# AO33/HiC_Genome_Assembler

Hardware: AMD Instinct MI355X
Metric: Part1+Part2 wall-clock (s) and bins/s on N x N contact map (higher is better)
Workload: dtype f64

## Files before the change

hic_genome_assembler_amd/csrc/k_part2_window.hip:

```cpp
#include <cstdlib>

#include "hicmi_internal.h"

namespace hicmi {

__device__ __forceinline__ double wave_sum_w(double v)
{
#pragma unroll
    for (int off = 32; off >= 1; off >>= 1) v += __shfl_xor(v, off, 64);
    return v;
}

static constexpr int WT_SLICES = 64;
static constexpr int WT_UNIT = 160;
__host__ __device__ inline int64_t wt_q_size(int k) { return ((int64_t)k * 2) << k; }
__host__ __device__ inline int64_t wt_p_size(int k) { return ((int64_t)k * k * 4) << k; }
int64_t window_table_doubles(int k) { return WT_SLICES * wt_q_size(k) + wt_p_size(k) + 8; }

__host__ __device__ inline void wt_split(int Lj, int m, int n_out, int& nrg, int& nq)
{
    const int nr = Lj > 0 ? (Lj + 15) >> 4 : 1, tiles_w = ((((m + 15) >> 4) + 3) >> 2);
    const int64_t work = (int64_t)nr * tiles_w * ((n_out + 3) >> 2);
    int64_t units = (work + WT_UNIT - 1) / WT_UNIT;
    units = units < 1 ? 1 : (units > WT_SLICES ? WT_SLICES : units);
    nrg = nr < (int)units ? nr : (int)units;
    nq = (int)units / nrg;
    const int by_cols = n_out >= 64 ? n_out / 32 : 1;
    nq = nq > by_cols ? by_cols : nq;
    nq = nq < 1 ? 1 : nq;
}

static constexpr int WT_ACC = 8;

__device__ __forceinline__ int spread_bit(int v, int b) { return ((v >> b) << (b + 1)) | (v & ((1 << b) - 1)); }

template <bool H_IN_LDS>
__global__ __launch_bounds__(256) void k_win_outside(const double* __restrict__ M2, int64_t ld2,
                                                     const int32_t* __restrict__ pos2sel, int n, int k,
                                                     const WindowBatchEntry* __restrict__ wb, const double* H,
                                                     double* __restrict__ tables, int64_t table_stride)
{
    extern __shared__ __attribute__((aligned(16))) unsigned char smem_w[];
    __shared__ int s_len[8], s_glen[256];
    const WindowBatchEntry& we = wb[blockIdx.y];
    const int j = blockIdx.x, p0 = we.p0, m = we.m;
    const int tid = threadIdx.x, lane = tid & 63, wave = tid >> 6;
    int nrg, nq;
    wt_split(we.w.len[j], m, n - m, nrg, nq);
    if ((int)blockIdx.z >= nrg * nq) return;
    if (tid < k) s_len[tid] = we.w.len[tid];
    const double hn = H[n - 1];
    if (H_IN_LDS) {
        double* hl = reinterpret_cast<double*>(smem_w);
        for (int i = tid; i < n; i += 256) hl[i] = H[i];
        H = hl;
    }
    __syncthreads();
    if (tid < (1 << k)) {
        int g = 0;
        for (int b = 0; b < k; b++) if ((tid >> b) & 1) g += s_len[b];
        s_glen[tid] = g;
    }
    __syncthreads();
    const int Lj = s_len[j], startj = we.w.start[j], n_out = n - m;
    const int rt = blockIdx.z % nrg, qs = blockIdx.z / nrg;
    const int q_lo = (int)(((int64_t)qs * n_out) / nq), q_hi = (int)(((int64_t)(qs + 1) * n_out) / nq);
    double* __restrict__ Q = tables + (int64_t)blockIdx.y * table_stride + blockIdx.z * wt_q_size(k) + (((int64_t)j * 2) << k);
    const int n_entries = 2 << (k - 1);
    for (int e0 = wave * WT_ACC; e0 < n_entries; e0 += 4 * WT_ACC) {
        double acc[WT_ACC];
        int off[WT_ACC], rev[WT_ACC];
#pragma unroll
        for (int u = 0; u < WT_ACC; u++) {
            const int e = e0 + u < n_entries ? e0 + u : n_entries - 1;
            rev[u] = e >> (k - 1);
            off[u] = p0 + s_glen[spread_bit(e & ((1 << (k - 1)) - 1), j)];
            acc[u] = 0.0;
        }
        for (int i = rt * 16; i < Lj; i = (i & 15) == 15 ? i + 1 + (nrg - 1) * 16 : i + 1) {
            const double* __restrict__ row = M2 + (int64_t)(startj + i) * ld2;
#pragma unroll 2
            for (int qq = q_lo + lane; qq < q_hi; qq += 64) {
                const int pos = qq < p0 ? qq : qq + m;
                const double v = row[pos2sel[pos]];
#pragma unroll
                for (int u = 0; u < WT_ACC; u++) {
                    const int slot = off[u] + (rev[u] ? Lj - 1 - i : i);
                    const int d = slot > pos ? slot - pos : pos - slot;
                    acc[u] += v * (hn - H[d - 1]);
                }
            }
        }
#pragma unroll
        for (int u = 0; u < WT_ACC; u++) {
            const double sum = wave_sum_w(acc[u]);
            const int e = e0 + u;
            if (lane == 0 && e < n_entries)
                Q[((int64_t)(e >> (k - 1)) << k) | spread_bit(e & ((1 << (k - 1)) - 1), j)] = sum;
        }
    }
}

typedef double mfma_d4 __attribute__((ext_vector_type(4)));
static constexpr int WM_QC = 128;
static constexpr int WM_MAX_TILES = 8;

template <bool H_IN_LDS, int TILES>
__global__ __launch_bounds__(256) void k_win_outside_mfma(const double* __restrict__ M2, int64_t ld2,
                                                          const int32_t* __restrict__ pos2sel, int n, int k,
                                                          const WindowBatchEntry* __restrict__ wb, const double* H,
                                                          double* __restrict__ tables, int64_t table_stride, int m_pad_max)
{
    extern __shared__ __attribute__((aligned(16))) unsigned char smem_w[];
    double* As = reinterpret_cast<double*>(smem_w);
    double* Gt = As;
    const int as_doubles = 16 * (WM_QC + 1) > 16 * m_pad_max ? 16 * (WM_QC + 1) : 16 * m_pad_max;
    __shared__ int s_len[8], s_glen[256], s_pos[WM_QC], s_col[WM_QC];
    const WindowBatchEntry& we = wb[blockIdx.y];
    const int j = blockIdx.x, p0 = we.p0, m = we.m;
    const int tid = threadIdx.x, lane = tid & 63, wave = tid >> 6;
    int nrg, nq;
    wt_split(we.w.len[j], m, n - m, nrg, nq);
    if ((int)blockIdx.z >= nrg * nq) return;
    if (tid < k) s_len[tid] = we.w.len[tid];
    const double hn = H[n - 1];
    if (H_IN_LDS) {
        double* hl = As + as_doubles;
        for (int i = tid; i < n; i += 256) hl[i] = H[i];
        H = hl;
    }
    __syncthreads();
    if (tid < (1 << k)) {
        int g = 0;
        for (int b = 0; b < k; b++) if ((tid >> b) & 1) g += s_len[b];
        s_glen[tid] = g;
    }
    __syncthreads();
    const int Lj = s_len[j], startj = we.w.start[j], n_out = n - m;
    const int rt = blockIdx.z % nrg, qs = blockIdx.z / nrg;
    const int q_lo = (int)(((int64_t)qs * n_out) / nq), q_hi = (int)(((int64_t)(qs + 1) * n_out) / nq);
    double* __restrict__ Q = tables + (int64_t)blockIdx.y * table_stride + blockIdx.z * wt_q_size(k) + (((int64_t)j * 2) << k);
    const int n_entries = 2 << (k - 1);
    const int m_pad = (m + 15) & ~15, n_tiles = m_pad >> 4;
    const int e_rev = tid < n_entries ? tid >> (k - 1) : 0;
    const int e_off = tid < n_entries ? s_glen[spread_bit(tid & ((1 << (k - 1)) - 1), j)] : 0;
    double qacc = 0.0;
    for (int r0 = rt * 16; r0 < Lj; r0 += nrg * 16) {
        mfma_d4 acc[TILES];
#pragma unroll
        for (int t = 0; t < TILES; t++) acc[t] = mfma_d4{0.0, 0.0, 0.0, 0.0};
        for (int qc = q_lo; qc < q_hi; qc += WM_QC) {
            const int cols = q_hi - qc < WM_QC ? q_hi - qc : WM_QC;
            if (q_hi - q_lo > WM_QC || r0 == rt * 16) {
                __syncthreads();
                if (tid < WM_QC) {
                    const int qq = qc + tid;
                    const int pos = tid < cols ? (qq < p0 ? qq : qq + m) : -1;
                    s_pos[tid] = pos;
                    s_col[tid] = pos >= 0 ? pos2sel[pos] : 0;
                }
            }
            __syncthreads();
            {
                constexpr int RPT = 16 * WM_QC / 256;
                const int cq = tid % WM_QC, rb = (tid / WM_QC) * RPT;
                const int c = s_col[cq];
                const bool okc = cq < cols;
                double v[RPT];
#pragma unroll
                for (int r = 0; r < RPT; r++)
                    v[r] = okc && r0 + rb + r < Lj ? M2[(int64_t)(startj + r0 + rb + r) * ld2 + c] : 0.0;
#pragma unroll
                for (int r = 0; r < RPT; r++) As[(rb + r) * (WM_QC + 1) + cq] = v[r];
            }
            __syncthreads();
            const int kk_end = (cols + 3) >> 2;
#pragma unroll 2
            for (int kk = 0; kk < kk_end; kk++) {
                const int kq = kk * 4 + (lane >> 4);
                const double a = As[(lane & 15) * (WM_QC + 1) + kq];
                int pos = s_pos[kq];
                pos = pos < 0 ? p0 : pos;
#pragma unroll
                for (int t = 0; t < TILES; t++) {
                    const int st = wave + 4 * t;
                    if (st < n_tiles) {
                        int d = p0 + st * 16 + (lane & 15) - pos;
                        d = d < 0 ? -d : d;
                        d = d < 1 ? 1 : (d > n - 1 ? n - 1 : d);
                        const double b = hn - H[d - 1];
                        acc[t] = __builtin_amdgcn_mfma_f64_16x16x4f64(a, b, acc[t], 0, 0, 0);
                    }
                }
            }
        }
        __syncthreads();
#pragma unroll
        for (int t = 0; t < TILES; t++) {
            const int st = wave + 4 * t;
            if (st < n_tiles) {
#pragma unroll
                for (int r = 0; r < 4; r++) Gt[((lane >> 4) + 4 * r) * m_pad_max + st * 16 + (lane & 15)] = acc[t][r];
            }
        }
        __syncthreads();
        if (tid < n_entries) {
            const int rows = Lj - r0 < 16 ? Lj - r0 : 16;
            for (int r = 0; r < rows; r++) {
                const int i = r0 + r;
                qacc += Gt[r * m_pad_max + e_off + (e_rev ? Lj - 1 - i : i)];
            }
        }
        __syncthreads();
    }
    if (tid < n_entries) Q[((int64_t)e_rev << k) | spread_bit(tid & ((1 << (k - 1)) - 1), j)] = qacc;
}

template <bool H_IN_LDS>
__global__ __launch_bounds__(256) void k_win_pairs(const double* __restrict__ M2, int64_t ld2, int n, int k,
                                                   const WindowBatchEntry* __restrict__ wb, const double* H,
                                                   double* __restrict__ tables, int64_t table_stride)
{
    extern __shared__ __attribute__((aligned(16))) unsigned char smem_w[];
    __shared__ int s_len[8], s_glen[256];
    __shared__ double s_part[4];
    const WindowBatchEntry& we = wb[blockIdx.y];
    const int a = blockIdx.x / k, b = blockIdx.x - a * k, m = we.m;
    const int tid = threadIdx.x, lane = tid & 63, wave = tid >> 6;
    if (tid < k) s_len[tid] = we.w.len[tid];
    const double hn = H[n - 1];
    if (H_IN_LDS) {
        double* hl = reinterpret_cast<double*>(smem_w);
        for (int i = tid; i < m; i += 256) hl[i] = H[i];
        H = hl;
    }
    __syncthreads();
    if (tid < (1 << k)) {
        int g = 0;
        for (int c = 0; c < k; c++) if ((tid >> c) & 1) g += s_len[c];
        s_glen[tid] = g;
    }
    __syncthreads();
    double* __restrict__ base = tables + (int64_t)blockIdx.y * table_stride;
    const int La = s_len[a], starta = we.w.start[a];
    if (a == b) {
        double acc = 0.0;
        const int pairs = La * La;
        for (int flat = tid; flat < pairs; flat += 256) {
            const int e = flat / La, f = flat - e * La;
            if (f > e) acc += M2[(int64_t)(starta + e) * ld2 + starta + f] * (hn - H[f - e - 1]);
        }
        acc = wave_sum_w(acc);
        if (lane == 0) s_part[wave] = acc;
        __syncthreads();
        if (tid == 0) base[WT_SLICES * wt_q_size(k) + wt_p_size(k) + a] = (s_part[0] + s_part[1]) + (s_part[2] + s_part[3]);
        int nrg, nq;
        wt_split(La, m, n - m, nrg, nq);
        const int nz = nrg * nq;
        const int64_t q_size = wt_q_size(k);
        for (int e = tid; e < (2 << k) && nz > 1; e += 256) {
            if ((e >> a) & 1) continue;
            double* __restrict__ q0 = base + (((int64_t)a * 2) << k) + e;
            double sum = q0[0];
            for (int z = 1; z < nz; z++) sum += q0[z * q_size];
            q0[0] = sum;
        }
        return;
    }
    const int Lb = s_len[b], startb = we.w.start[b];
    const int lo = a < b ? a : b, hi = a < b ? b : a;
    double* __restrict__ P = base + WT_SLICES * wt_q_size(k) + ((((int64_t)a * k + b) * 4) << k);
    const int n_sets = k >= 2 ? 1 << (k - 2) : 1, n_entries = 4 * n_sets, pairs = La * Lb;
    for (int e0 = wave * WT_ACC; e0 < n_entries; e0 += 4 * WT_ACC) {
        double acc[WT_ACC];
        int gap[WT_ACC], ra[WT_ACC], rb[WT_ACC];
#pragma unroll
        for (int u = 0; u < WT_ACC; u++) {
            const int e = e0 + u < n_entries ? e0 + u : n_entries - 1;
            const int orient = e / n_sets, set = e - orient * n_sets;
            ra[u] = orient >> 1; rb[u] = orient & 1;
            gap[u] = s_glen[spread_bit(spread_bit(set, lo), hi)];
            acc[u] = 0.0;
        }
#pragma unroll 2
        for (int flat = lane; flat < pairs; flat += 64) {
            const int ea = flat / Lb, eb = flat - ea * Lb;
            const double v = M2[(int64_t)(starta + ea) * ld2 + startb + eb];
#pragma unroll
            for (int u = 0; u < WT_ACC; u++) {
                const int i = ra[u] ? La - 1 - ea : ea, jj = rb[u] ? Lb - 1 - eb : eb;
                const int d = La - i + gap[u] + jj;
                acc[u] += v * (hn - H[d - 1]);
            }
        }
#pragma unroll
        for (int u = 0; u < WT_ACC; u++) {
            const double sum = wave_sum_w(acc[u]);
            const int e = e0 + u;
            if (lane == 0 && e < n_entries) {
                const int orient = e / n_sets, set = e - orient * n_sets;
                P[((int64_t)orient << k) | spread_bit(spread_bit(set, lo), hi)] = sum;
            }
        }
    }
}

__global__ __launch_bounds__(256) void k_win_candidates(int k, const int8_t* __restrict__ orders,
                                                        const uint8_t* __restrict__ orients, int n_ori, int n_cand,
                                                        const double* __restrict__ tables, int64_t table_stride,
                                                        double* __restrict__ delta_all)
{
    const int c = blockIdx.x * 256 + threadIdx.x;
    if (c >= n_cand) return;
    const double* __restrict__ base = tables + (int64_t)blockIdx.y * table_stride;
    const double* __restrict__ Q = base;
    const int64_t q_size = wt_q_size(k);
    const double* __restrict__ P = base + WT_SLICES * q_size;
    const double* __restrict__ C = P + wt_p_size(k);
    const int8_t* __restrict__ ord = orders + (int64_t)(c / n_ori) * k;
    const uint8_t* __restrict__ ori = orients + (int64_t)(c % n_ori) * k;
    double sum = 0.0;
    for (int j = 0; j < k; j++) sum += C[j];
    int before = 0;
    for (int s = 0; s < k; s++) {
        const int a = ord[s], ra = ori[s] ? 1 : 0;
        const int64_t qi = ((int64_t)(a * 2 + ra) << k) | before;
        sum += Q[qi];
        int between = 0;
        for (int t = s + 1; t < k; t++) {
            const int b = ord[t], rb = ori[t] ? 1 : 0;
            sum += P[((((int64_t)a * k + b) * 4 + ra * 2 + rb) << k) | between];
            between |= 1 << b;
        }
        before |= 1 << a;
    }
    delta_all[(int64_t)blockIdx.y * n_cand + c] = sum;
}

static constexpr int NL_ITERS = 32;
static constexpr int NL_ORDERS = 4 * NL_ITERS;
static inline int64_t stride_of(int k) { return window_table_doubles(k); }

template <bool LIST>
__global__ __launch_bounds__(256) void k_win_near(int k, const int8_t* __restrict__ orders, const uint8_t* __restrict__ orients,
                                                  int n_ord, int n_ori, const double* __restrict__ tables, int64_t table_stride,
                                                  const WindowBatchEntry* __restrict__ wb, int whole, double total, double cur_fast,
                                                  double floor, double near_top, double* __restrict__ part,
                                                  int32_t* __restrict__ count, NearEntry* __restrict__ near, int cap)
{
    __shared__ double s_stage[4][128];
    __shared__ int s_omask[256];
    __shared__ int s_ps[28], s_pt[28];
    __shared__ double s_red[4];
    __shared__ double s_c[3];
    __shared__ int s_any;
    const int tid = threadIdx.x, lane = tid & 63, wave = tid >> 6, win = blockIdx.y;
    const double* __restrict__ Q = tables + (int64_t)win * table_stride;
    const double* __restrict__ P = Q + WT_SLICES * wt_q_size(k);
    const double* __restrict__ C = P + wt_p_size(k);
    const int npairs = k * (k - 1) / 2, n_stage = 2 * k + 4 * npairs;
    for (int oi = tid; oi < n_ori; oi += 256) {
        int m = 0;
        for (int s = 0; s < k; s++) if (orients[(int64_t)oi * k + s]) m |= 1 << s;
        s_omask[oi] = m;
    }
    if (tid == 0) {
        int p = 0;
        for (int s = 0; s < k; s++)
            for (int t = s + 1; t < k; t++) { s_ps[p] = s; s_pt[p] = t; p++; }
        double sum = 0.0;
        for (int j = 0; j < k; j++) sum += C[j];
        s_c[0] = sum;
        const uint8_t* __restrict__ ori = orients + (int64_t)wb[win].c0 * k;
        int before = 0;
        for (int s = 0; s < k; s++) {
            const int ra = ori[s] ? 1 : 0;
            sum += Q[((int64_t)(s * 2 + ra) << k) | before];
            int between = 0;
            for (int t = s + 1; t < k; t++) {
                const int rb = ori[t] ? 1 : 0;
                sum += P[((((int64_t)s * k + t) * 4 + ra * 2 + rb) << k) | between];
                between |= 1 << t;
            }
            before |= 1 << s;
        }
        s_c[1] = sum;
    }
    if (LIST) {
        double v = -INFINITY;
        for (int b = tid; b < (int)gridDim.x; b += 256) v = fmax(v, part[(int64_t)win * gridDim.x + b]);
#pragma unroll
        for (int off = 32; off >= 1; off >>= 1) v = fmax(v, __shfl_xor(v, off, 64));
        if (lane == 0) s_red[wave] = v;
        __syncthreads();
        if (tid == 0) {
            const double mx = fmax(fmax(s_red[0], s_red[1]), fmax(s_red[2], s_red[3]));
            s_any = mx > -INFINITY;
            const double top = mx > floor ? mx : floor;
            s_c[2] = top - fabs(top) * near_top;
        }
    }
    __syncthreads();
    if (LIST && !s_any) return;
    const double sumC = s_c[0], d0 = s_c[1], thr = LIST ? s_c[2] : 0.0;
    double vmax = -INFINITY;
    double* __restrict__ st = s_stage[wave];
    for (int it = 0; it < NL_ITERS; it++) {
        const int o = blockIdx.x * NL_ORDERS + it * 4 + wave;
        const bool live = o < n_ord;
        if (live) {
            const int8_t* __restrict__ ord = orders + (int64_t)o * k;
            int a_[8];
#pragma unroll
            for (int t = 0; t < 8; t++) a_[t] = t < k ? ord[t] : 0;
            for (int e = lane; e < n_stage; e += 64) {
                double v;
                if (e < 2 * k) {
                    const int s = e >> 1, r = e & 1;
                    int a = 0, before = 0;
#pragma unroll
                    for (int t = 0; t < 8; t++) { if (t < s) before |= 1 << a_[t]; if (t == s) a = a_[t]; }
                    v = Q[((int64_t)(a * 2 + r) << k) | before];
                } else {
                    const int p = (e - 2 * k) >> 2, rr = (e - 2 * k) & 3, s = s_ps[p], t = s_pt[p];
                    int a = 0, b = 0, between = 0;
#pragma unroll
                    for (int u = 0; u < 8; u++) {
                        if (u == s) a = a_[u];
                        if (u == t) b = a_[u];
                        if (u > s && u < t) between |= 1 << a_[u];
                    }
                    v = P[((((int64_t)a * k + b) * 4 + rr) << k) | between];
                }
                st[e] = v;
            }
        }
        __syncthreads();
        if (live) {
            for (int oi = lane; oi < n_ori; oi += 64) {
                const int om = s_omask[oi];
                double sum = sumC;
                int p4 = 2 * k;
                for (int s = 0; s < k; s++) {
                    const int rs = (om >> s) & 1;
                    sum += st[2 * s + rs];
                    for (int t = s + 1; t < k; t++, p4 += 4) sum += st[p4 + rs * 2 + ((om >> t) & 1)];
                }
                const double f = whole ? sum / total : cur_fast + (sum - d0) / total;
                if (!__builtin_isfinite(f)) continue;
                if (!LIST) vmax = fmax(vmax, f);
                else if (f >= thr) {
                    const int slot = atomicAdd(count + win, 1);
                    if (slot < cap) {
                        NearEntry& ne = near[(int64_t)win * cap + slot];
                        ne.cand = o * n_ori + oi; ne.pad = 0; ne.fast = f;
                    }
                }
            }
        }
        __syncthreads();
    }
    if (!LIST) {
#pragma unroll
        for (int off = 32; off >= 1; off >>= 1) vmax = fmax(vmax, __shfl_xor(vmax, off, 64));
        if (lane == 0) s_red[wave] = vmax;
        __syncthreads();
        if (tid == 0) part[(int64_t)win * gridDim.x + blockIdx.x] = fmax(fmax(s_red[0], s_red[1]), fmax(s_red[2], s_red[3]));
    }
}

static std::atomic<int> g_lds_out{0}, g_lds_pairs{0};

static void build_window_tables(const double* M2, int64_t ld2, const int32_t* pos2sel, int n, int k,
                                const WindowBatchEntry* wb, const WindowBatchEntry* h_wb, int n_win, int max_m,
                                const double* H, double* tables, hipStream_t s)
{
    const int64_t stride = window_table_doubles(k);
    const size_t h_all = (((size_t)n * sizeof(double)) + 15) & ~(size_t)15;
    const size_t h_win = (((size_t)max_m * sizeof(double)) + 15) & ~(size_t)15;
    const int m_pad_max = (max_m + 15) & ~15;
    int n_slices = 1;
    for (int w = 0; w < n_win; w++)
        for (int j = 0; j < k; j++) {
            int nrg, nq;
            wt_split(h_wb[w].w.len[j], h_wb[w].m, n - h_wb[w].m, nrg, nq);
            n_slices = nrg * nq > n_slices ? nrg * nq : n_slices;
        }
    const size_t lds_mfma = (size_t)16 * (size_t)(WM_QC + 1 > m_pad_max ? WM_QC + 1 : m_pad_max) * sizeof(double);
    static const bool valu_only = getenv("HICMI_P2_WINDOW_VALU") != nullptr;
    if (!valu_only && m_pad_max <= 16 * 4 * WM_MAX_TILES && k <= 8) {
        const bool h_lds = lds_mfma + h_all <= 150 * 1024;
        const size_t lds = lds_mfma + (h_lds ? h_all : 0);
        const int tiles = m_pad_max <= 128 ? 2 : (m_pad_max <= 256 ? 4 : 8);
#define HICMI_WIN_MFMA(HL, T)                                                                                                   \
        do {                                                                                                                    \
            static std::atomic<int> lds_set{0};                                                                                 \
            ensure_dynamic_lds(reinterpret_cast<const void*>(k_win_outside_mfma<HL, T>), lds_set, lds);                         \
            hipLaunchKernelGGL((k_win_outside_mfma<HL, T>), dim3(k, n_win, n_slices), dim3(256), lds, s, M2, ld2, pos2sel, n, k, \
                               wb, H, tables, stride, m_pad_max);                                                               \
        } while (0)
        if (h_lds) { if (tiles == 2) HICMI_WIN_MFMA(true, 2); else if (tiles == 4) HICMI_WIN_MFMA(true, 4); else HICMI_WIN_MFMA(true, 8); }
        else       { if (tiles == 2) HICMI_WIN_MFMA(false, 2); else if (tiles == 4) HICMI_WIN_MFMA(false, 4); else HICMI_WIN_MFMA(false, 8); }
#undef HICMI_WIN_MFMA
    }
    else if (h_all <= 96 * 1024) {
        ensure_dynamic_lds(reinterpret_cast<const void*>(k_win_outside<true>), g_lds_out, h_all);
        hipLaunchKernelGGL(k_win_outside<true>, dim3(k, n_win, n_slices), dim3(256), h_all, s, M2, ld2, pos2sel, n, k, wb, H, tables, stride);
    } else {
        hipLaunchKernelGGL(k_win_outside<false>, dim3(k, n_win, n_slices), dim3(256), 0, s, M2, ld2, pos2sel, n, k, wb, H, tables, stride);
    }
    if (h_win <= 96 * 1024) {
        ensure_dynamic_lds(reinterpret_cast<const void*>(k_win_pairs<true>), g_lds_pairs, h_win);
        hipLaunchKernelGGL(k_win_pairs<true>, dim3(k * k, n_win), dim3(256), h_win, s, M2, ld2, n, k, wb, H, tables, stride);
    } else {
        hipLaunchKernelGGL(k_win_pairs<false>, dim3(k * k, n_win), dim3(256), 0, s, M2, ld2, n, k, wb, H, tables, stride);
    }
}

void launch_p2_window_tables(const double* M2, int64_t ld2, const int32_t* pos2sel, int n, int k,
                             const WindowBatchEntry* wb, const WindowBatchEntry* h_wb, int n_win, int max_m, const double* H,
                             double* tables, hipStream_t s)
{
    if (n_win <= 0 || k < 1) return;
    build_window_tables(M2, ld2, pos2sel, n, k, wb, h_wb, n_win, max_m, H, tables, s);
}

void launch_p2_window_candidates(int k, int n_win, const int8_t* orders, const uint8_t* orients, int n_ord, int n_ori,
                                 const double* tables, double* delta_all, hipStream_t s)
{
    if (n_win <= 0 || k < 1) return;
    const int n_cand = n_ord * n_ori;
    hipLaunchKernelGGL(k_win_candidates, dim3((n_cand + 255) / 256, n_win), dim3(256), 0, s, k, orders, orients, n_ori, n_cand,
                       tables, stride_of(k), delta_all);
}

int window_near_blocks(int n_ord) { return (n_ord + NL_ORDERS - 1) / NL_ORDERS; }

void launch_p2_window_near(const double* M2, int64_t ld2, const int32_t* pos2sel, int n, int k,
                           const WindowBatchEntry* wb, const WindowBatchEntry* h_wb, int n_win, int max_m, const int8_t* orders,
                           const uint8_t* orients, int n_ord, int n_ori, const double* H, double* tables, int whole, double total,
                           double cur_fast, double floor, double near_top, double* part, int32_t* count, NearEntry* near, int cap,
                           hipStream_t s)
{
    if (n_win <= 0 || k < 1 || k > 8) return;
    build_window_tables(M2, ld2, pos2sel, n, k, wb, h_wb, n_win, max_m, H, tables, s);
    const dim3 grid(window_near_blocks(n_ord), n_win);
    hipLaunchKernelGGL(k_win_near<false>, grid, dim3(256), 0, s, k, orders, orients, n_ord, n_ori, (const double*)tables,
                       stride_of(k), wb, whole, total, cur_fast, floor, near_top, part, count, near, cap);
    (void)hipMemsetAsync(count, 0, sizeof(int32_t) * (size_t)n_win, s);
    hipLaunchKernelGGL(k_win_near<true>, grid, dim3(256), 0, s, k, orders, orients, n_ord, n_ori, (const double*)tables,
                       stride_of(k), wb, whole, total, cur_fast, floor, near_top, part, count, near, cap);
}

}
```

Before: 120,200.

## Add diagonal-binning kernel for window outside-contact tables

Adds a new kernel for the window Q tables, made the default path for narrow windows. It reduces each row-block tile of the contact map into per-diagonal bins, two tiles at a time with double buffering, then takes a dot product of the bins with a distance-weight vector. This replaces the previous per-entry MFMA path. A separate work split feeds the pairs kernel's slice reduction, and the old MFMA path stays reachable through an environment variable. This is meant to remove the redundant per-entry matrix work, at the cost of more LDS use and a different summation order.

```diff
diff --git a/hic_genome_assembler_amd/csrc/k_part2_window.hip b/hic_genome_assembler_amd/csrc/k_part2_window.hip
--- a/hic_genome_assembler_amd/csrc/k_part2_window.hip
+++ b/hic_genome_assembler_amd/csrc/k_part2_window.hip
@@ -216,10 +216,177 @@
     if (tid < n_entries) Q[((int64_t)e_rev << k) | spread_bit(tid & ((1 << (k - 1)) - 1), j)] = qacc;
 }
 
+static constexpr int WD_C = 512;
+static constexpr int WD_TILES = 4;
+
+__host__ __device__ inline void wd_split(int Lj, int n_out, int& nrg, int& nq)
+{
+    const int nr = Lj > 0 ? (Lj + 15) >> 4 : 1, ct = (n_out + WM_QC - 1) / WM_QC;
+    int64_t units = ((int64_t)nr * ct + WD_TILES - 1) / WD_TILES;
+    units = units < 1 ? 1 : (units > WT_SLICES ? WT_SLICES : units);
+    const int by_cols = n_out >= 2 * WM_QC ? n_out / WM_QC : (n_out >= 64 ? 2 : 1);
+    units = units < 2 && by_cols >= 2 ? 2 : units;
+    nq = (int)units < by_cols ? (int)units : by_cols;
+    nrg = (int)units / nq;
+    nrg = nrg > nr ? nr : nrg;
+    nrg = nrg < 1 ? 1 : nrg;
+}
+
+__device__ __forceinline__ void wd_slice(int qs, int nq, int p0, int n_out, int& q_lo, int& q_hi)
+{
+    const int nl = p0 < n_out ? p0 : n_out, nrt = n_out - nl;
+    if (nq < 2 || nl == 0 || nrt == 0) {
+        q_lo = (int)(((int64_t)qs * n_out) / nq); q_hi = (int)(((int64_t)(qs + 1) * n_out) / nq);
+        return;
+    }
+    int nql = (int)(((int64_t)nq * nl + n_out / 2) / n_out);
+    nql = nql < 1 ? 1 : (nql > nq - 1 ? nq - 1 : nql);
+    if (qs < nql) { q_lo = (int)(((int64_t)qs * nl) / nql); q_hi = (int)(((int64_t)(qs + 1) * nl) / nql); }
+    else {
+        const int r = qs - nql, nqr = nq - nql;
+        q_lo = nl + (int)(((int64_t)r * nrt) / nqr); q_hi = nl + (int)(((int64_t)(r + 1) * nrt) / nqr);
+    }
+}
+
+__host__ __device__ inline void wt_split_of(bool diag, int Lj, int m, int n_out, int& nrg, int& nq)
+{
+    if (diag) wd_split(Lj, n_out, nrg, nq);
+    else wt_split(Lj, m, n_out, nrg, nq);
+}
+
+static constexpr int WD_PAD = 15, WD_TS = WM_QC + 2 * WD_PAD + 1;
+static size_t wd_lds_bytes(int m_cap) { return sizeof(double) * (size_t)(2 * 16 * WD_TS + 3 * WD_C + 3 * m_cap); }
+
+__global__ __launch_bounds__(256) void k_win_outside_diag(const double* __restrict__ M2, int64_t ld2,
+                                                          const int32_t* __restrict__ pos2sel, int n, int k,
+                                                          const WindowBatchEntry* __restrict__ wb, const double* __restrict__ H,
+                                                          double* __restrict__ tables, int64_t table_stride, int m_cap)
+{
+    extern __shared__ __attribute__((aligned(16))) unsigned char smem_w[];
+    constexpr int TS = WD_TS;
+    double* tile = reinterpret_cast<double*>(smem_w);
+    double* bins0 = tile + 2 * 16 * TS;
+    double* bins1 = bins0 + WD_C + m_cap;
+    double* wl = bins1 + WD_C + m_cap;
+    __shared__ double s_dot[256];
+    const WindowBatchEntry& we = wb[blockIdx.y];
+    const int j = blockIdx.x, p0 = we.p0, m = we.m, Lj = we.w.len[j], startj = we.w.start[j];
+    const int tid = threadIdx.x, n_out = n - m;
+    int nrg, nq;
+    wd_split(Lj, n_out, nrg, nq);
+    if ((int)blockIdx.z >= nrg * nq) return;
+    const double hn = H[n - 1];
+    const int rt = blockIdx.z % nrg, qs = blockIdx.z / nrg;
+    int q_lo, q_hi;
+    wd_slice(qs, nq, p0, n_out, q_lo, q_hi);
+    const int nr = Lj > 0 ? (Lj + 15) >> 4 : 1, LjP = nr * 16, nra = (nr - rt + nrg - 1) / nrg;
+    const int E = 1 << k, G = 256 >> k, e = tid & (E - 1), g = tid >> k;
+    const int e_rev = e >> (k - 1), e_set = spread_bit(e & ((1 << (k - 1)) - 1), j);
+    int cB = p0;
+    for (int b = 0; b < k; b++) if ((e_set >> b) & 1) cB += we.w.len[b];
+    const int cq = tid & (WM_QC - 1), rb = (tid / WM_QC) * 8;
+    const int half = tid >> 7, bt_lo = tid & 127;
+    for (int i = tid; i < 2 * 16 * (TS - WM_QC); i += 256) {
+        const int row = i / (TS - WM_QC), c = i - row * (TS - WM_QC);
+        tile[row * TS + (c < WD_PAD ? c : c + WM_QC)] = 0.0;
+    }
+    double qacc = 0.0;
+    for (int part = 0; part < 2; part++) {
+        const int s_lo = part == 0 ? q_lo : (q_lo > p0 ? q_lo : p0);
+        const int s_hi = part == 0 ? (q_hi < p0 ? q_hi : p0) : q_hi;
+        for (int c0 = s_lo; c0 < s_hi && Lj > 0; c0 += WD_C) {
+            const int Cc = s_hi - c0 < WD_C ? s_hi - c0 : WD_C;
+            const int pos_lo = part == 0 ? c0 : c0 + m;
+            const int ntc = (Cc + WM_QC - 1) / WM_QC;
+            for (int i = tid; i < ntc * WM_QC + LjP; i += 256) { bins0[i] = 0.0; bins1[i] = 0.0; }
+            const int xmin = p0 - pos_lo - Cc + 1, nx = Cc + m - 1;
+            for (int i = tid; i < nx; i += 256) {
+                int d = xmin + i;
+                d = d < 0 ? -d : d;
+                d = d < 1 ? 1 : (d > n - 1 ? n - 1 : d);
+                wl[i] = hn - H[d - 1];
+            }
+            const int T = nra * ntc;
+            auto load_tile = [&](int s, double (&v)[8]) {
+                if (s >= T) return;
+                const int a = s / ntc, t0 = (s - a * ntc) * WM_QC, r0 = (rt + a * nrg) * 16 + rb;
+                const int c = t0 + cq < Cc ? pos2sel[pos_lo + t0 + cq] : -1;
+#pragma unroll
+                for (int r = 0; r < 8; r++) v[r] = c >= 0 && r0 + r < Lj ? M2[(int64_t)(startj + r0 + r) * ld2 + c] : 0.0;
+            };
+            auto store_tile = [&](int s, const double (&v)[8]) {
+                if (s >= T) return;
+                double* __restrict__ tn = tile + (s & 1) * 16 * TS + WD_PAD;
+#pragma unroll
+                for (int r = 0; r < 8; r++) tn[(rb + r) * TS + cq] = v[r];
+            };
+            auto reduce_tile = [&](int s) {
+                const double* __restrict__ tb = tile + (s & 1) * 16 * TS;
+                const int a = s / ntc, t0 = (s - a * ntc) * WM_QC, r0 = (rt + a * nrg) * 16;
+                for (int bt = bt_lo; bt < WM_QC + 15; bt += 128) {
+                    double x[16];
+                    if (half == 0) {
+#pragma unroll
+                        for (int r = 0; r < 16; r++) x[r] = tb[r * TS + bt + r];
+                    } else {
+#pragma unroll
+                        for (int r = 0; r < 16; r++) x[r] = tb[r * TS + WD_PAD + bt - r];
+                    }
+                    double sum = 0.0;
+#pragma unroll
+                    for (int r = 0; r < 16; r++) sum += x[r];
+                    if (half == 0) bins0[t0 - r0 + bt - 15 + LjP - 1] += sum;
+                    else bins1[t0 + r0 + bt] += sum;
+                }
+            };
+            double va[8], vb[8];
+            load_tile(0, va);
+            load_tile(1, vb);
+            store_tile(0, va);
+            load_tile(2, va);
+            __syncthreads();
+            for (int s = 0; s < T; s += 2) {
+                reduce_tile(s);
+                store_tile(s + 1, vb);
+                load_tile(s + 3, vb);
+                __syncthreads();
+                if (s + 1 < T) {
+                    reduce_tile(s + 1);
+                    store_tile(s + 2, va);
+                    load_tile(s + 4, va);
+                    __syncthreads();
+                }
+            }
+            const double* __restrict__ bp = e_rev ? bins1 : bins0;
+            const int wi = (e_rev ? cB + Lj - 1 - pos_lo : cB - pos_lo + LjP - 1) - xmin;
+            const int hi = e_rev ? Cc + Lj - 1 : Cc + LjP - 1;
+            int idx = (e_rev ? 0 : LjP - Lj) + g;
+            double acc = 0.0;
+            for (; idx + 7 * G < hi; idx += 8 * G) {
+                double bv[8], wv[8];
+#pragma unroll
+                for (int u = 0; u < 8; u++) { bv[u] = bp[idx + u * G]; wv[u] = wl[wi - idx - u * G]; }
+#pragma unroll
+                for (int u = 0; u < 8; u++) acc += bv[u] * wv[u];
+            }
+            for (; idx < hi; idx += G) acc += bp[idx] * wl[wi - idx];
+            s_dot[tid] = acc;
+            __syncthreads();
+            if (tid < E) {
+                double sum = 0.0;
+                for (int gg = 0; gg < G; gg++) sum += s_dot[gg * E + tid];
+                qacc += sum;
+            }
+        }
+    }
+    if (tid < E)
+        tables[(int64_t)blockIdx.y * table_stride + blockIdx.z * wt_q_size(k) + (((int64_t)j * 2) << k) + (((int64_t)e_rev << k) | e_set)] = qacc;
+}
+
 template <bool H_IN_LDS>
 __global__ __launch_bounds__(256) void k_win_pairs(const double* __restrict__ M2, int64_t ld2, int n, int k,
                                                    const WindowBatchEntry* __restrict__ wb, const double* H,
-                                                   double* __restrict__ tables, int64_t table_stride)
+                                                   double* __restrict__ tables, int64_t table_stride, int diag_split)
 {
     extern __shared__ __attribute__((aligned(16))) unsigned char smem_w[];
     __shared__ int s_len[8], s_glen[256];
@@ -255,7 +422,7 @@
         __syncthreads();
         if (tid == 0) base[WT_SLICES * wt_q_size(k) + wt_p_size(k) + a] = (s_part[0] + s_part[1]) + (s_part[2] + s_part[3]);
         int nrg, nq;
-        wt_split(La, m, n - m, nrg, nq);
+        wt_split_of(diag_split != 0, La, m, n - m, nrg, nq);
         const int nz = nrg * nq;
         const int64_t q_size = wt_q_size(k);
         for (int e = tid; e < (2 << k) && nz > 1; e += 256) {
@@ -479,16 +646,27 @@
     const size_t h_all = (((size_t)n * sizeof(double)) + 15) & ~(size_t)15;
     const size_t h_win = (((size_t)max_m * sizeof(double)) + 15) & ~(size_t)15;
     const int m_pad_max = (max_m + 15) & ~15;
+    static const bool valu_only = getenv("HICMI_P2_WINDOW_VALU") != nullptr;
+    static const bool mfma_only = getenv("HICMI_P2_WINDOW_MFMA") != nullptr;
+    const bool narrow = m_pad_max <= 16 * 4 * WM_MAX_TILES && k <= 8;
+    const bool diag = narrow && !valu_only && !mfma_only;
     int n_slices = 1;
     for (int w = 0; w < n_win; w++)
         for (int j = 0; j < k; j++) {
             int nrg, nq;
-            wt_split(h_wb[w].w.len[j], h_wb[w].m, n - h_wb[w].m, nrg, nq);
+            wt_split_of(diag, h_wb[w].w.len[j], h_wb[w].m, n - h_wb[w].m, nrg, nq);
             n_slices = nrg * nq > n_slices ? nrg * nq : n_slices;
         }
     const size_t lds_mfma = (size_t)16 * (size_t)(WM_QC + 1 > m_pad_max ? WM_QC + 1 : m_pad_max) * sizeof(double);
-    static const bool valu_only = getenv("HICMI_P2_WINDOW_VALU") != nullptr;
-    if (!valu_only && m_pad_max <= 16 * 4 * WM_MAX_TILES && k <= 8) {
+    if (diag) {
+        static std::atomic<int> lds_set{0};
+        const int m_cap = m_pad_max < 16 ? 16 : m_pad_max;
+        const size_t lds = wd_lds_bytes(m_cap);
+        ensure_dynamic_lds(reinterpret_cast<const void*>(k_win_outside_diag), lds_set, lds);
+        hipLaunchKernelGGL(k_win_outside_diag, dim3(k, n_win, n_slices), dim3(256), lds, s, M2, ld2, pos2sel, n, k, wb, H, tables,
+                           stride, m_cap);
+    }
+    else if (!valu_only && narrow) {
         const bool h_lds = lds_mfma + h_all <= 150 * 1024;
         const size_t lds = lds_mfma + (h_lds ? h_all : 0);
         const int tiles = m_pad_max <= 128 ? 2 : (m_pad_max <= 256 ? 4 : 8);
@@ -511,9 +689,9 @@
     }
     if (h_win <= 96 * 1024) {
         ensure_dynamic_lds(reinterpret_cast<const void*>(k_win_pairs<true>), g_lds_pairs, h_win);
-        hipLaunchKernelGGL(k_win_pairs<true>, dim3(k * k, n_win), dim3(256), h_win, s, M2, ld2, n, k, wb, H, tables, stride);
+        hipLaunchKernelGGL(k_win_pairs<true>, dim3(k * k, n_win), dim3(256), h_win, s, M2, ld2, n, k, wb, H, tables, stride, (int)diag);
     } else {
-        hipLaunchKernelGGL(k_win_pairs<false>, dim3(k * k, n_win), dim3(256), 0, s, M2, ld2, n, k, wb, H, tables, stride);
+        hipLaunchKernelGGL(k_win_pairs<false>, dim3(k * k, n_win), dim3(256), 0, s, M2, ld2, n, k, wb, H, tables, stride, (int)diag);
     }
 }
 
```

After: 123,400 (median of 6 runs). 1.03x the previous value.
